# leonardsiegert/PULPo

Measured on AMD Instinct MI355X. Metric: volume-pairs/sec fwd+bwd, 160^3 fp32, higher is better.
Workload: dtype f32

## Files before the change

pulpo_amd/csrc/resample.hip:

```cpp
#include "act_io.h"

namespace {

template <int VEC, typename T = float>
__global__ __launch_bounds__(256) void avgpool2_fwd_kernel(const T* __restrict__ in, long ips, T* __restrict__ out, long ops, int B,
                                                             int D, int H, int W, int Do, int Ho, int Wo, int C) {
    const int CV = C / VEC;
    const long total = (long)B * Do * Ho * Wo * CV;
    for (long e = blockIdx.x * (long)blockDim.x + threadIdx.x; e < total; e += (long)gridDim.x * blockDim.x) {
        const int c = (int)(e % CV) * VEC;
        long p = e / CV;
        const int ox = (int)(p % Wo); p /= Wo;
        const int oy = (int)(p % Ho); p /= Ho;
        const int oz = (int)(p % Do);
        const int b = (int)(p / Do);
        const int z1 = min(2 * oz + 2, D), y1 = min(2 * oy + 2, H), x1 = min(2 * ox + 2, W);
        float acc[VEC];
#pragma unroll
        for (int k = 0; k < VEC; ++k) acc[k] = 0.f;
        for (int z = 2 * oz; z < z1; ++z)
            for (int y = 2 * oy; y < y1; ++y)
                for (int x = 2 * ox; x < x1; ++x) {
                    float t[VEC];
                    pulpo::ldv<VEC>(in + ((((long)b * D + z) * H + y) * W + x) * ips + c, t);
// ... 161 lines not shown
        const int z = (int)(p % Di);
        const long pl = p / Di;
        int zl, zh, yl, yh, xl, xh;
        gather_window(z, sd, Do, zl, zh);
        gather_window(y, sh, Ho, yl, yh);
        gather_window(x, sw, Wo, xl, xh);
        const float* g = gout + pl * (long)Do * Ho * Wo;
        float acc = 0.f;
        for (int oz = zl; oz <= zh; ++oz) {
            const float wz = gather_weight(oz, z, sd, Di);
            if (wz == 0.f) continue;
            for (int oy = yl; oy <= yh; ++oy) {
                const float wy = gather_weight(oy, y, sh, Hi);
                if (wy == 0.f) continue;
                float row = 0.f;
                for (int ox = xl; ox <= xh; ++ox) {
                    const float wx = gather_weight(ox, x, sw, Wi);
                    if (wx != 0.f) row += g[((long)oz * Ho + oy) * Wo + ox] * mult * wx;
                }
                acc += row * (wz * wy);
            }
        }
        gin[e] = acc;
    }
}

__device__ __forceinline__ float up2_weight(int o, int m, int in_size) {
    int i0, i1;
    float lam;
    src_index(o, 0.5f, in_size, i0, i1, lam);
    return (i0 == m ? 1.f - lam : 0.f) + (i1 == m ? lam : 0.f);
}

__global__ __launch_bounds__(256) void resize_up2_bwd_kernel(const float* __restrict__ gout, float* __restrict__ gin, long nplanes, int Di, int Hi,
                                                               int Wi, float mult) {
    const int Do = 2 * Di, Ho = 2 * Hi, Wo = 2 * Wi;
    const long total = nplanes * Di * Hi * Wi;
    for (long e = blockIdx.x * (long)blockDim.x + threadIdx.x; e < total; e += (long)gridDim.x * blockDim.x) {
        long p = e;
        const int x = (int)(p % Wi); p /= Wi;
        const int y = (int)(p % Hi); p /= Hi;
        const int z = (int)(p % Di);
        const long pl = p / Di;
        const float* g = gout + pl * (long)Do * Ho * Wo;
        float wz4[4], wy4[4], wx4[4];
#pragma unroll
        for (int k = 0; k < 4; ++k) {
            const int oz = 2 * z - 1 + k, oy = 2 * y - 1 + k, ox = 2 * x - 1 + k;
            wz4[k] = (oz >= 0 && oz < Do) ? up2_weight(oz, z, Di) : 0.f;
            wy4[k] = (oy >= 0 && oy < Ho) ? up2_weight(oy, y, Hi) : 0.f;
            wx4[k] = (ox >= 0 && ox < Wo) ? up2_weight(ox, x, Wi) : 0.f;
        }
        float acc = 0.f;
#pragma unroll
        for (int kz = 0; kz < 4; ++kz) {
            const int oz = 2 * z - 1 + kz;
            if (oz < 0 || oz >= Do) continue;
#pragma unroll
            for (int ky = 0; ky < 4; ++ky) {
                const int oy = 2 * y - 1 + ky;
                if (oy < 0 || oy >= Ho) continue;
                const float wzy = wz4[kz] * wy4[ky];
                const float* row = g + ((long)oz * Ho + oy) * Wo;
#pragma unroll
                for (int kx = 0; kx < 4; ++kx) {
                    const int ox = 2 * x - 1 + kx;
                    if (ox >= 0 && ox < Wo) acc += wzy * wx4[kx] * row[ox];
                }
            }
        }
        gin[e] = acc * mult;
    }
}

constexpr int kMaxSrc = 8;
struct FeedbackArgs {
    const float* src[kMaxSrc];
    float* gsrc[kMaxSrc];
    int ch[kMaxSrc];
    int nsrc, ctot;
    int B, Di, Hi, Wi;
};

template <typename T = float>
__global__ __launch_bounds__(256) void feedback_fwd_kernel(FeedbackArgs a, T* __restrict__ out, long ops) {
    const int Do = 2 * a.Di, Ho = 2 * a.Hi, Wo = 2 * a.Wi;
    const long Vi = (long)a.Di * a.Hi * a.Wi;
    const long total = (long)a.B * Do * Ho * Wo;
    for (long e = blockIdx.x * (long)blockDim.x + threadIdx.x; e < total; e += (long)gridDim.x * blockDim.x) {
        long p = e;
        const int ox = (int)(p % Wo); p /= Wo;
        const int oy = (int)(p % Ho); p /= Ho;
        const int oz = (int)(p % Do);
        const int b = (int)(p / Do);
        int z0, z1, y0, y1, x0, x1;
        float lz, ly, lx;
        src_index(oz, 0.5f, a.Di, z0, z1, lz);
        src_index(oy, 0.5f, a.Hi, y0, y1, ly);
        src_index(ox, 0.5f, a.Wi, x0, x1, lx);
        const long o00 = ((long)z0 * a.Hi + y0) * a.Wi, o01 = ((long)z0 * a.Hi + y1) * a.Wi;
        const long o10 = ((long)z1 * a.Hi + y0) * a.Wi, o11 = ((long)z1 * a.Hi + y1) * a.Wi;
        const float wz0 = 1.f - lz, wy0 = 1.f - ly, wx0 = 1.f - lx;
        T* d = out + e * ops;
        int cc = 0;
        for (int s = 0; s < a.nsrc; ++s) {
// ... 176 lines not shown
                                     int C, void* stream) {
    PULPO_REQUIRE(add != nullptr, "avgpool2_bwd_add: null pointer");
    return pulpo_avgpool2_bwd_t(gout, gops, add, aps, gin, gips, 0, B, D, H, W, C, stream);
}

PULPO_API int pulpo_resize_trilinear_scaled_fwd(const float* in, const float* add, float* out, int64_t nplanes, int Di, int Hi, int Wi, int Do, int Ho,
                                                int Wo, float scale_d, float scale_h, float scale_w, float mult, void* stream) {
    PULPO_REQUIRE(in && out && nplanes > 0 && Di > 0 && Hi > 0 && Wi > 0 && Do > 0 && Ho > 0 && Wo > 0, "resize_fwd: bad arguments");
    const float sd = scale_d > 0.f ? scale_d : (float)Di / (float)Do, sh = scale_h > 0.f ? scale_h : (float)Hi / (float)Ho,
                sw = scale_w > 0.f ? scale_w : (float)Wi / (float)Wo;
    if (Do == 2 * Di && Ho == 2 * Hi && Wo == 2 * Wi && sd == 0.5f && sh == 0.5f && sw == 0.5f && nplanes * (long)Do * Ho < (1L << 31) &&
        (((uintptr_t)out | (uintptr_t)add) & 7) == 0) {
        hipLaunchKernelGGL(resize_up2_fwd_kernel, dim3(eblocks(nplanes * Do * Ho * Wi)), dim3(256), 0, (hipStream_t)stream, in, add, out, (int)nplanes, Di, Hi,
                           Wi, mult);
        return pulpo::check_launch("resize_up2_fwd");
    }
    hipLaunchKernelGGL(resize_fwd_kernel, dim3(eblocks(nplanes * Do * Ho * Wo)), dim3(256), 0, (hipStream_t)stream, in, add, out, (long)nplanes, Di,
                       Hi, Wi, Do, Ho, Wo, sd, sh, sw, mult);
    return pulpo::check_launch("resize_fwd");
}

PULPO_API int pulpo_resize_trilinear_fwd(const float* in, const float* add, float* out, int64_t nplanes, int Di, int Hi, int Wi, int Do, int Ho, int Wo,
                                         float mult, void* stream) {
    return pulpo_resize_trilinear_scaled_fwd(in, add, out, nplanes, Di, Hi, Wi, Do, Ho, Wo, 0.f, 0.f, 0.f, mult, stream);
}

static int resize_bwd_impl(const float* gout, float* gin, int64_t nplanes, int Di, int Hi, int Wi, int Do, int Ho, int Wo,
                           float scale_d, float scale_h, float scale_w, float mult, bool det, void* stream) {
    PULPO_REQUIRE(gout && gin && nplanes > 0 && Di > 0 && Hi > 0 && Wi > 0 && Do > 0 && Ho > 0 && Wo > 0, "resize_bwd: bad arguments");
    hipStream_t st = (hipStream_t)stream;
    const float sd = scale_d > 0.f ? scale_d : (float)Di / (float)Do, sh = scale_h > 0.f ? scale_h : (float)Hi / (float)Ho,
                sw = scale_w > 0.f ? scale_w : (float)Wi / (float)Wo;
    if (Do == 2 * Di && Ho == 2 * Hi && Wo == 2 * Wi && sd == 0.5f && sh == 0.5f && sw == 0.5f) {
        hipLaunchKernelGGL(resize_up2_bwd_kernel, dim3(eblocks(nplanes * Di * Hi * Wi)), dim3(256), 0, st, gout, gin, (long)nplanes, Di, Hi, Wi, mult);
        return pulpo::check_launch("resize_up2_bwd");
    }
    if (det) {
        hipLaunchKernelGGL(resize_bwd_gather_kernel, dim3(eblocks(nplanes * Di * Hi * Wi)), dim3(256), 0, st, gout, gin, (long)nplanes, Di, Hi, Wi, Do,
                           Ho, Wo, sd, sh, sw, mult);
        return pulpo::check_launch("resize_bwd_gather");
    }
    hipError_t e = hipMemsetAsync(gin, 0, sizeof(float) * nplanes * Di * Hi * Wi, st);
    if (e != hipSuccess) return pulpo::fail((int)e, "resize_bwd memset: %s", hipGetErrorString(e));
    hipLaunchKernelGGL(resize_bwd_atomic_kernel, dim3(eblocks(nplanes * Do * Ho * Wo)), dim3(256), 0, st, gout, gin, (long)nplanes, Di, Hi, Wi, Do,
                       Ho, Wo, sd, sh, sw, mult);
    return pulpo::check_launch("resize_bwd_atomic");
}

PULPO_API int pulpo_resize_trilinear_scaled_bwd(const float* gout, float* gin, int64_t nplanes, int Di, int Hi, int Wi, int Do, int Ho, int Wo,
                                                float scale_d, float scale_h, float scale_w, float mult, void* stream) {
    return resize_bwd_impl(gout, gin, nplanes, Di, Hi, Wi, Do, Ho, Wo, scale_d, scale_h, scale_w, mult, false, stream);
}

PULPO_API int pulpo_resize_trilinear_scaled_bwd_det(const float* gout, float* gin, int64_t nplanes, int Di, int Hi, int Wi, int Do, int Ho, int Wo,
                                                    float scale_d, float scale_h, float scale_w, float mult, void* stream) {
    return resize_bwd_impl(gout, gin, nplanes, Di, Hi, Wi, Do, Ho, Wo, scale_d, scale_h, scale_w, mult, true, stream);
}

PULPO_API int pulpo_resize_trilinear_bwd(const float* gout, float* gin, int64_t nplanes, int Di, int Hi, int Wi, int Do, int Ho, int Wo, float mult,
                                         void* stream) {
    return pulpo_resize_trilinear_scaled_bwd(gout, gin, nplanes, Di, Hi, Wi, Do, Ho, Wo, 0.f, 0.f, 0.f, mult, stream);
}

PULPO_API int pulpo_feedback_up2_fwd_t(const float* const* srcs, const int* chans, int nsrc, void* out, int dt, int64_t ops, int B, int Di, int Hi,
                                       int Wi, void* stream) {
    PULPO_REQUIRE(srcs && chans && out && nsrc > 0 && nsrc <= kMaxSrc && B > 0, "feedback_up2_fwd: bad arguments");
    PULPO_REQUIRE_DT(dt, "feedback_up2_fwd");
// ... 37 lines not shown
```

pulpo_amd/csrc/warp.hip:

```cpp
#include "common.h"
#include "sampling.h"

namespace {

using pulpo::Corner;
using pulpo::sample_coord;

template <int C>
__global__ __launch_bounds__(256) void warp_fwd_kernel(const float* __restrict__ df, const float* __restrict__ img, const float* __restrict__ add,
                                                         float* __restrict__ out, int B, int Dg, int Hg, int Wg, int Di, int Hi, int Wi, int Cr) {
    const long Vg = (long)Dg * Hg * Wg, Vi = (long)Di * Hi * Wi;
    const long total = (long)B * Vg;
    const int nch = C > 0 ? C : Cr;
    for (long e = blockIdx.x * (long)blockDim.x + threadIdx.x; e < total; e += (long)gridDim.x * blockDim.x) {
        const long b = B == 1 ? 0 : e / Vg, v = e - b * Vg;
        const int vi = (int)v;
        const int x = vi % Wg, y = (vi / Wg) % Hg, z = vi / (Wg * Hg);
        const float* d = df + b * 3 * Vg + v;
        const Corner cz = sample_coord((float)z, d[0], Dg, Di);
        const Corner cy = sample_coord((float)y, d[Vg], Hg, Hi);
        const Corner cx = sample_coord((float)x, d[2 * Vg], Wg, Wi);
        const long o00 = ((long)cz.i0 * Hi + cy.i0) * Wi, o01 = ((long)cz.i0 * Hi + cy.i1) * Wi;
        const long o10 = ((long)cz.i1 * Hi + cy.i0) * Wi, o11 = ((long)cz.i1 * Hi + cy.i1) * Wi;
        const float wz0 = 1.f - cz.f, wy0 = 1.f - cy.f, wx0 = 1.f - cx.f;
// ... 197 lines not shown
                const Corner cy = sample_coord((float)y, fld[V + vox], H, H);
                const Corner cx = sample_coord((float)x, fld[2 * V + vox], W, W);
                const int o00 = (cz.i0 * H + cy.i0) * W, o01 = (cz.i0 * H + cy.i1) * W;
                const int o10 = (cz.i1 * H + cy.i0) * W, o11 = (cz.i1 * H + cy.i1) * W;
                const float wz0 = 1.f - cz.f, wy0 = 1.f - cy.f, wx0 = 1.f - cx.f;
#pragma unroll
                for (int c = 0; c < 3; ++c) {
                    const float* s = fld + c * V;
                    float val = wz0 * wy0 * wx0 * s[o00 + cx.i0] + wz0 * wy0 * cx.f * s[o00 + cx.i1] + wz0 * cy.f * wx0 * s[o01 + cx.i0] +
                                wz0 * cy.f * cx.f * s[o01 + cx.i1] + cz.f * wy0 * wx0 * s[o10 + cx.i0] + cz.f * wy0 * cx.f * s[o10 + cx.i1] +
                                cz.f * cy.f * wx0 * s[o11 + cx.i0] + cz.f * cy.f * cx.f * s[o11 + cx.i1];
                    val += s[vox];
                    nv[j][c] = val;
                }
            }
        }
        __syncthreads();
        float* out = work + (long)(k + 1) * n + b * 3 * V;
#pragma unroll
        for (int j = 0; j < 8; ++j) {
            const int vox = tid + j * VI_THREADS;
            if (vox < V) {
#pragma unroll
                for (int c = 0; c < 3; ++c) {
                    fld[c * V + vox] = nv[j][c];
                    out[c * V + vox] = nv[j][c];
                }
            }
        }
        __syncthreads();
    }
}

inline int eblocks(long items) { return (int)std::max<long>(1, std::min<long>((items + 255) / 256, 8192)); }

__device__ __forceinline__ double fx_unit(const unsigned* maxbits) {
    const float m = __uint_as_float(*maxbits);
    if (!(m > 0.f) || !(m < INFINITY)) return 1.0;
    int ex;
    frexpf(m, &ex);
    return ldexp(1.0, 46 - ex);
}
__device__ __forceinline__ void fx_add(long long* p, float v, double unit) {
    atomicAdd(reinterpret_cast<unsigned long long*>(p), (unsigned long long)__double2ll_rn((double)v * unit));
}

__device__ __forceinline__ void block_absmax_to(float m, unsigned* out) {
    __shared__ float wm[4];
#pragma unroll
    for (int o = 32; o > 0; o >>= 1) m = fmaxf(m, __shfl_xor(m, o, 64));
    if ((threadIdx.x & 63) == 0) wm[threadIdx.x >> 6] = m;
    __syncthreads();
    if (threadIdx.x == 0) {
        const float t = fmaxf(fmaxf(wm[0], wm[1]), fmaxf(wm[2], wm[3]));
        if (t > 0.f) atomicMax(out, __float_as_uint(t));
    }
}
inline int fx_blocks(long items) { return (int)std::max<long>(1, std::min<long>((items + 255) / 256, 1024)); }

__global__ __launch_bounds__(256) void absmax_kernel(const float* __restrict__ g, long n, unsigned* __restrict__ out) {
    float m = 0.f;
    for (long e = blockIdx.x * (long)blockDim.x + threadIdx.x; e < n; e += (long)gridDim.x * blockDim.x) m = fmaxf(m, fabsf(g[e]));
    block_absmax_to(m, out);
}

template <bool SELF>
// ... 98 lines not shown
    hipStream_t st = (hipStream_t)stream;
    const long n = (long)B * 3 * D * H * W, total = (long)B * D * H * W;
    constexpr long VECINT_LDS_MAXV = 2048;
    static_assert(VECINT_LDS_MAXV <= VI_MAXV, "the one-launch form holds the whole field in LDS");
    if (total / B <= VECINT_LDS_MAXV && nsteps > 0) {
        const size_t lds = sizeof(float) * 3 * (size_t)(total / B);
        static bool attr_set = false;
        if (!attr_set) {
            hipError_t e = hipFuncSetAttribute(reinterpret_cast<const void*>(&vecint_fwd_lds_kernel), hipFuncAttributeMaxDynamicSharedMemorySize,
                                               (int)(sizeof(float) * 3 * VI_MAXV));
            if (e != hipSuccess) return pulpo::fail((int)e, "hipFuncSetAttribute(vecint_fwd_lds): %s", hipGetErrorString(e));
            attr_set = true;
        }
        hipLaunchKernelGGL(vecint_fwd_lds_kernel, dim3(B), dim3(VI_THREADS), lds, st, v, work, B, D, H, W, nsteps, 1.0f / (float)(1 << nsteps));
        return pulpo::check_launch("vecint_fwd_lds");
    }
    hipLaunchKernelGGL(scale_kernel, dim3(eblocks(n)), dim3(256), 0, st, v, work, 1.0f / (float)(1 << nsteps), n);
    int rc = pulpo::check_launch("vecint scale");
    if (rc) return rc;
    for (int k = 0; k < nsteps; ++k) {
        const float* cur = work + (long)k * n;
        hipLaunchKernelGGL(warp_fwd_kernel<3>, dim3(eblocks(total)), dim3(256), 0, st, cur, cur, cur, work + (long)(k + 1) * n, B, D, H, W, D, H, W, 3);
        rc = pulpo::check_launch("vecint step");
        if (rc) return rc;
    }
    return 0;
}

static bool vecint_bwd_tiled(int D, int H, int W) {
    constexpr int TILED_MIN = 8;
    return D >= TILED_MIN && H >= TILED_MIN && W >= TILED_MIN;
}

PULPO_API size_t pulpo_vecint_bwd_tmp_floats(int B, int D, int H, int W, int nsteps) {
    if (B <= 0 || D < 1 || H < 1 || W < 1 || nsteps <= 0) return 0;
    const size_t n = (size_t)B * 3 * D * H * W;
    return vecint_bwd_tiled(D, H, W) ? (size_t)nsteps * n : 2 * n;
}

PULPO_API int pulpo_vecint_bwd(const float* work, const float* gout, float* gin, float* tmp, int B, int D, int H, int W, int nsteps, void* stream) {
    PULPO_REQUIRE(work && gout && gin && B > 0 && D >= 1 && H > 1 && W > 1 && nsteps >= 0 && (long)D * H * W < (1L << 31), "vecint_bwd: bad arguments");
    PULPO_REQUIRE(tmp || pulpo_vecint_bwd_tmp_floats(B, D, H, W, nsteps) == 0, "vecint_bwd: scratch of pulpo_vecint_bwd_tmp_floats() floats required");
    hipStream_t st = (hipStream_t)stream;
    const long n = (long)B * 3 * D * H * W, total = (long)B * D * H * W;
    const float scale = 1.0f / (float)(1 << nsteps);
    const bool tiled = vecint_bwd_tiled(D, H, W);
    if (tiled && nsteps > 0) {
        hipError_t e = hipMemsetAsync(tmp, 0, sizeof(float) * n * nsteps, st);
        if (e != hipSuccess) return pulpo::fail((int)e, "vecint_bwd fill: %s", hipGetErrorString(e));
    }
    const float* g = gout;
    for (int k = nsteps - 1; k >= 0; --k) {
        const float* cur = work + (long)k * n;
        float* gp;
        if (tiled) {
            gp = tmp + (long)k * n;
            const int ntz = pulpo::cdiv(D, 4), nty = pulpo::cdiv(H, 8), ntx = pulpo::cdiv(W, 8);
            if (k == nsteps - 1 && (long)D * H * W >= 64L * 64 * 64)
                hipLaunchKernelGGL(vecint_bwd_tile_kernel<2>, dim3((unsigned)((long)B * ntz * nty * ntx)), dim3(256), 0, st, cur, g, gp, B, D, H, W, ntz, nty, ntx);
            else
                hipLaunchKernelGGL(vecint_bwd_tile_kernel<1>, dim3((unsigned)((long)B * ntz * nty * ntx)), dim3(256), 0, st, cur, g, gp, B, D, H, W, ntz, nty, ntx);
        } else {
            gp = tmp + (long)(k & 1) * n;
            hipError_t e = hipMemcpyAsync(gp, g, sizeof(float) * n, hipMemcpyDeviceToDevice, st);
            if (e != hipSuccess) return pulpo::fail((int)e, "vecint_bwd copy: %s", hipGetErrorString(e));
            hipLaunchKernelGGL(warp_bwd_kernel<true>, dim3(eblocks(total)), dim3(256), 0, st, cur, cur, g, gp, gp, B, D, H, W, D, H, W, 3);
        }
        int rc = pulpo::check_launch("vecint_bwd step");
        if (rc) return rc;
        g = gp;
    }
    hipLaunchKernelGGL(scale_kernel, dim3(eblocks(n)), dim3(256), 0, st, g, gin, scale, n);
    return pulpo::check_launch("vecint_bwd scale");
}

PULPO_API size_t pulpo_warp3d_bwd_det_ws_bytes(int B, int C, int Di, int Hi, int Wi) {
    if (B <= 0 || C <= 0 || Di < 1 || Hi < 1 || Wi < 1) return 0;
    return 256 + sizeof(long long) * (size_t)B * C * Di * Hi * Wi;
// ... 56 lines not shown
```

pulpo_amd/csrc/conv3d_wino3.hip:

```cpp
#include "conv_shared.h"
#include "wino3_pack.h"

namespace {

using namespace pulpo_conv;
using f32x2 = __attribute__((ext_vector_type(2))) float;

constexpr int Q_CH = 8, Q_NT = 32;
constexpr int Q_PL = HY * 4;
constexpr int Q_PLROWS = 4 * Q_PL + 2;
constexpr int Q_QROWS = 6 * Q_PLROWS;
constexpr int Q_IMG = 2 * Q_QROWS * 4;
static_assert((2 * Q_PLROWS) % 16 == 4 && (Q_QROWS * 4) % 32 == 16, "bank layout");
constexpr int Q_NITEM = 6 * HY * 4 * 2;
constexpr int Q_TAB = 3 * 512;
constexpr int Q_R = 8 * 2 * 16 * 64;
constexpr int Q_RED = 8 * 2 * Q_NT;
constexpr int Q_PART = 8 * 64 * 8;
constexpr size_t Q_LDS = (size_t)(2 * Q_IMG + Q_TAB + Q_R + Q_RED + Q_PART) * sizeof(float);
static_assert(Q_LDS <= 160 * 1024, "one workgroup per CU");


template <bool BNR, int SP>
__device__ __forceinline__ void wino3_body(const ConvArgs& a) {
// ... 204 lines not shown
                    acc[s0 >> 2][s0 & 3] = __builtin_amdgcn_mfma_f32_32x32x2f32(av0[s2], wv0[s2], acc[s0 >> 2][s0 & 3], 0, 0, 0);
                    acc[s1 >> 2][s1 & 3] = __builtin_amdgcn_mfma_f32_32x32x2f32(av1[s2], wv1[s2], acc[s1 >> 2][s1 & 3], 0, 0, 0);
                    if (s2 == 0) {
                        __builtin_amdgcn_sched_barrier(0);
                        if (pp == SP) {
                            store_item(img_w);
                            if (chunk + 2 == nchunk) halo_offsets(has_next ? nxt : cur);
                        }
                        if (pp == SP + 1) { load_raw(st_rs, st_c0, 0); load_raw(st_rs, st_c0, 1); load_raw(st_rs, st_c0, 2); load_raw(st_rs, st_c0, 3); }
                        __builtin_amdgcn_sched_barrier(0);
                    }
                    if (s2 == 1 && pp + 1 < 4) {
                        __builtin_amdgcn_sched_barrier(0);
                        combine(avn0, avn1);
                        __builtin_amdgcn_sched_barrier(0);
                        if (pp + 2 < 4) fetch_a(pp + 2);
                        __builtin_amdgcn_sched_barrier(0);
                    }
                }
                wr[pp & 1][0] = pp < 2 ? load_w(wcur, s0 + 2) : load_w(wnext, s0 - 2);
                wr[pp & 1][1] = pp < 2 ? load_w(wcur, s1 + 2) : load_w(wnext, s1 - 2);
                __builtin_amdgcn_sched_barrier(0);
            }
            wcur += w_chunk_stride;
            __syncthreads();
            cb ^= 1;
            if (chunk == 0) flush_stats();
        }

        float* out_b = a.out + (long)cur.b * a.out_bs;
        const int z0 = cur.z0, y0 = cur.y0, x0 = cur.x0, co0 = cur.co0;
        int elane = lane;
        asm volatile("" : "+v"(elane));
        const int q = elane & 7, kh = (elane >> 3) & 1, g = elane >> 4;
        const float4 zero4 = make_float4(0.f, 0.f, 0.f, 0.f);
        float4 s4 = zero4, q4 = zero4;
        const bool fuse = !BNR && a.coef != nullptr;
        const float4 b4 = BNR ? zero4 : *reinterpret_cast<const float4*>(tab + co0 + 4 * q);
        const float4 bm4 = *reinterpret_cast<const float4*>(tab + co0 + 4 * q);
        const float4 sc4 = *reinterpret_cast<const float4*>(tab + ctab + co0 + 4 * q);
        const float4 sh4 = *reinterpret_cast<const float4*>(tab + 2 * ctab + co0 + 4 * q);
        const float* bn_b = BNR ? a.bn_y + (long)cur.b * a.bn_y_bs + co0 + 4 * q : nullptr;
        const int combo = wave * 4 + g;
        const int ox = combo >> 4, rr = combo & 15;
        const int row = (rr & 3) + 8 * (rr >> 2) + 4 * kh;
        const int vzb = row >> 4, vyb = (row >> 2) & 3, vxb = row & 3;
        float4 yv0 = zero4, yv1 = zero4;
        const bool qok = co0 + 4 * q < a.Cout;
        auto load_y = [&](int oz_) {
            if (BNR && qok) {
                const long vox_ = (long)((z0 + 2 * vzb + oz_) * a.H + y0 + 2 * vyb) * a.W + x0 + 2 * vxb + ox;
                yv0 = *reinterpret_cast<const float4*>(bn_b + vox_ * a.bn_y_ps);
                yv1 = *reinterpret_cast<const float4*>(bn_b + (vox_ + a.W) * a.bn_y_ps);
            }
        };
        load_y(0);
        __builtin_amdgcn_sched_barrier(0);
        f32x2 m1 = {-1.f, -1.f};
        asm volatile("" : "+s"(m1));
#pragma unroll
        for (int p = 0; p < 2; ++p)
#pragma unroll
            for (int r = 0; r < 16; r += 2) {
                const f32x2 a0 = {acc[p][0][r], acc[p][0][r + 1]}, a1 = {acc[p][1][r], acc[p][1][r + 1]};
                const f32x2 a2 = {acc[p][2][r], acc[p][2][r + 1]}, a3 = {acc[p][3][r], acc[p][3][r + 1]};
                const f32x2 o0 = (a0 + a1) + a2, o1 = __builtin_elementwise_fma(m1, a3, __builtin_elementwise_fma(m1, a2, a1));
                acc[p][0][r] = o0.x; acc[p][0][r + 1] = o0.y;
                acc[p][1][r] = o1.x; acc[p][1][r + 1] = o1.y;
            }
#pragma unroll
        for (int oz = 0; oz < 2; ++oz) {
            if (oz > 0) __syncthreads();
            float* const r0 = R + ((wave * 2 + 0) * 16) * 64 + elane;
            float* const r1 = R + ((wave * 2 + 1) * 16) * 64 + elane;
            if (pzh == 0) {
#pragma unroll
                for (int r = 0; r < 16; r += 2) {
                    const f32x2 u0 = f32x2{acc[0][0][r], acc[0][0][r + 1]} + f32x2{acc[1][0][r], acc[1][0][r + 1]};
                    const f32x2 u1 = f32x2{acc[0][1][r], acc[0][1][r + 1]} + f32x2{acc[1][1][r], acc[1][1][r + 1]};
                    r0[r * 64] = oz == 0 ? u0.x : acc[1][0][r]; r0[(r + 1) * 64] = oz == 0 ? u0.y : acc[1][0][r + 1];
                    r1[r * 64] = oz == 0 ? u1.x : acc[1][1][r]; r1[(r + 1) * 64] = oz == 0 ? u1.y : acc[1][1][r + 1];
                }
            } else {
#pragma unroll
                for (int r = 0; r < 16; r += 2) {
                    const f32x2 u0 = __builtin_elementwise_fma(m1, f32x2{acc[0][0][r], acc[0][0][r + 1]}, f32x2{acc[1][0][r], acc[1][0][r + 1]});
                    const f32x2 u1 = __builtin_elementwise_fma(m1, f32x2{acc[0][1][r], acc[0][1][r + 1]}, f32x2{acc[1][1][r], acc[1][1][r + 1]});
                    r0[r * 64] = oz == 0 ? acc[0][0][r] : u0.x; r0[(r + 1) * 64] = oz == 0 ? acc[0][0][r + 1] : u0.y;
                    r1[r * 64] = oz == 0 ? acc[0][1][r] : u1.x; r1[(r + 1) * 64] = oz == 0 ? acc[0][1][r + 1] : u1.y;
                }
            }
            const int gz = z0 + 2 * vzb + oz, gy = y0 + 2 * vyb, gx = x0 + 2 * vxb + ox;
            const long vox = (long)(gz * a.H + gy) * a.W + gx;
            __syncthreads();
            float4 t[4];
#pragma unroll
            for (int p = 0; p < 4; ++p) {
                const float4 u0 = *reinterpret_cast<const float4*>(R + (((0 * 4 + p) * 2 + ox) * 16 + rr) * 64 + kh * 32 + 4 * q);
                const float4 u1 = *reinterpret_cast<const float4*>(R + (((1 * 4 + p) * 2 + ox) * 16 + rr) * 64 + kh * 32 + 4 * q);
                t[p] = make_float4(u0.x + u1.x, u0.y + u1.y, u0.z + u1.z, u0.w + u1.w);
            }
            float4 v0 = make_float4(t[0].x + t[1].x + t[2].x + b4.x, t[0].y + t[1].y + t[2].y + b4.y, t[0].z + t[1].z + t[2].z + b4.z, t[0].w + t[1].w + t[2].w + b4.w);
            float4 v1 = make_float4(t[1].x - t[2].x - t[3].x + b4.x, t[1].y - t[2].y - t[3].y + b4.y, t[1].z - t[2].z - t[3].z + b4.z, t[1].w - t[2].w - t[3].w + b4.w);
            if (BNR) {
                auto red1 = [&](float dzv, float yy, float sc, float sh, float m32, float& s_, float& q_) {
                    const float bn = yy * sc + sh;
                    const float d = bn > 0.f ? dzv : dzv * a.slope;
                    s_ += d;
                    q_ = fmaf(d, yy - m32, q_);
                };
                red1(v0.x, yv0.x, sc4.x, sh4.x, bm4.x, s4.x, q4.x); red1(v0.y, yv0.y, sc4.y, sh4.y, bm4.y, s4.y, q4.y);
                red1(v0.z, yv0.z, sc4.z, sh4.z, bm4.z, s4.z, q4.z); red1(v0.w, yv0.w, sc4.w, sh4.w, bm4.w, s4.w, q4.w);
                red1(v1.x, yv1.x, sc4.x, sh4.x, bm4.x, s4.x, q4.x); red1(v1.y, yv1.y, sc4.y, sh4.y, bm4.y, s4.y, q4.y);
                red1(v1.z, yv1.z, sc4.z, sh4.z, bm4.z, s4.z, q4.z); red1(v1.w, yv1.w, sc4.w, sh4.w, bm4.w, s4.w, q4.w);
                if (oz == 0) { __builtin_amdgcn_sched_barrier(0); load_y(1); __builtin_amdgcn_sched_barrier(0); }
            } else {
                s4.x += v0.x + v1.x; s4.y += v0.y + v1.y; s4.z += v0.z + v1.z; s4.w += v0.w + v1.w;
                q4.x += v0.x * v0.x + v1.x * v1.x; q4.y += v0.y * v0.y + v1.y * v1.y; q4.z += v0.z * v0.z + v1.z * v1.z; q4.w += v0.w * v0.w + v1.w * v1.w;
            }
            if (fuse) {
                auto act = [&](float v, float sc, float sh) { const float tt = v * sc + sh; return tt > 0.f ? tt : tt * a.slope; };
                v0 = make_float4(act(v0.x, sc4.x, sh4.x), act(v0.y, sc4.y, sh4.y), act(v0.z, sc4.z, sh4.z), act(v0.w, sc4.w, sh4.w));
                v1 = make_float4(act(v1.x, sc4.x, sh4.x), act(v1.y, sc4.y, sh4.y), act(v1.z, sc4.z, sh4.z), act(v1.w, sc4.w, sh4.w));
            }
            float* obase = out_b + (long)((co0 + 4 * q) >> 3) * a.out_kb + ((4 * q) & 7);
            if (qok) {
                *reinterpret_cast<float4*>(obase + vox * a.out_ps) = v0;
                *reinterpret_cast<float4*>(obase + (vox + a.W) * a.out_ps) = v1;
            }
        }
        if (a.stats != nullptr) {
            float* pw_ = part + (wave * 64 + elane) * 8;
            *reinterpret_cast<float4*>(pw_) = s4;
            *reinterpret_cast<float4*>(pw_ + 4) = q4;
            const int c_ = elane & 31, wh_ = elane >> 5;
            const float* pr_ = part + (wave * 64 + (c_ >> 2)) * 8 + wh_ * 4 + (c_ & 3);
            float t_ = 0.f;
#pragma unroll
            for (int j = 0; j < 8; ++j) t_ += pr_[j * 64];
            red[(wave * 2 + wh_) * NT + c_] = t_;
        }
        pend_tile = cur.tile_lin; pend_co0 = co0;
        if (!has_next) break;
        cur = nxt;
        work = next_work;
    }
    __syncthreads();
    flush_stats();
}

template <bool BNR>
__global__ __launch_bounds__(512, 1) void conv3d_k3_wino3_mfma(ConvArgs a) {
    if (__builtin_amdgcn_readfirstlane(threadIdx.x >> 8) != 0) wino3_body<BNR, 2>(a);
    else wino3_body<BNR, 0>(a);
}

__global__ void pack_weight_wino3_kernel(const float* __restrict__ w, float* __restrict__ wp, int Cin, int Cout, int NPad, int dgrad, long total) {
    for (long e = blockIdx.x * (long)blockDim.x + threadIdx.x; e < total; e += (long)gridDim.x * blockDim.x)
        pulpo_conv::pack_wino3_one(w, wp, Cin, Cout, NPad, dgrad, e);
}

constexpr int WINO3_MIN_K = 16;

// ... 103 lines not shown
```

Baseline: 38.02.

## Tile up2 resize backward through LDS and fuse small-volume vecint backward

The 2x-upsample trilinear backward now runs one block per 4x8x8 coarse tile. Each block stages its fine-gradient halo in shared memory and gathers from there, instead of every thread issuing 64 global loads. Separately, for tiny volumes (at most 1024 voxels), the whole scaling-and-squaring backward runs in one block-per-batch kernel that keeps the field and gradients in LDS across all steps. This removes the per-step launches, the memset and the scratch buffer. The fused path only triggers for small volumes, and the tiled resize adds a barrier and halo-redundant loads.

Result: no change. 38.19, median of 6 (+0.5%).

```diff
diff --git a/pulpo_amd/csrc/resample.hip b/pulpo_amd/csrc/resample.hip
--- a/pulpo_amd/csrc/resample.hip
+++ b/pulpo_amd/csrc/resample.hip
@@ -217,45 +217,53 @@
     return (i0 == m ? 1.f - lam : 0.f) + (i1 == m ? lam : 0.f);
 }
 
-__global__ __launch_bounds__(256) void resize_up2_bwd_kernel(const float* __restrict__ gout, float* __restrict__ gin, long nplanes, int Di, int Hi,
-                                                               int Wi, float mult) {
+template <int TZ_, int TY_, int TX_>
+__global__ __launch_bounds__(TZ_* TY_* TX_) void resize_up2_bwd_kernel(const float* __restrict__ gout, float* __restrict__ gin, int Di, int Hi, int Wi,
+                                                                       int ntz, int nty, int ntx, float mult) {
+    constexpr int NT = TZ_ * TY_ * TX_, FY = 2 * TY_ + 2, FX = 2 * TX_ + 2, FV = (2 * TZ_ + 2) * FY * FX;
+    __shared__ float fine[FV];
     const int Do = 2 * Di, Ho = 2 * Hi, Wo = 2 * Wi;
-    const long total = nplanes * Di * Hi * Wi;
-    for (long e = blockIdx.x * (long)blockDim.x + threadIdx.x; e < total; e += (long)gridDim.x * blockDim.x) {
-        long p = e;
-        const int x = (int)(p % Wi); p /= Wi;
-        const int y = (int)(p % Hi); p /= Hi;
-        const int z = (int)(p % Di);
-        const long pl = p / Di;
-        const float* g = gout + pl * (long)Do * Ho * Wo;
-        float wz4[4], wy4[4], wx4[4];
-#pragma unroll
-        for (int k = 0; k < 4; ++k) {
-            const int oz = 2 * z - 1 + k, oy = 2 * y - 1 + k, ox = 2 * x - 1 + k;
-            wz4[k] = (oz >= 0 && oz < Do) ? up2_weight(oz, z, Di) : 0.f;
-            wy4[k] = (oy >= 0 && oy < Ho) ? up2_weight(oy, y, Hi) : 0.f;
-            wx4[k] = (ox >= 0 && ox < Wo) ? up2_weight(ox, x, Wi) : 0.f;
-        }
-        float acc = 0.f;
-#pragma unroll
-        for (int kz = 0; kz < 4; ++kz) {
-            const int oz = 2 * z - 1 + kz;
-            if (oz < 0 || oz >= Do) continue;
-#pragma unroll
-            for (int ky = 0; ky < 4; ++ky) {
-                const int oy = 2 * y - 1 + ky;
-                if (oy < 0 || oy >= Ho) continue;
-                const float wzy = wz4[kz] * wy4[ky];
-                const float* row = g + ((long)oz * Ho + oy) * Wo;
-#pragma unroll
-                for (int kx = 0; kx < 4; ++kx) {
-                    const int ox = 2 * x - 1 + kx;
-                    if (ox >= 0 && ox < Wo) acc += wzy * wx4[kx] * row[ox];
-                }
+    int t = blockIdx.x;
+    const int tx_ = t % ntx; t /= ntx;
+    const int ty_ = t % nty; t /= nty;
+    const int tz_ = t % ntz;
+    const long pl = t / ntz;
+    const int z0 = tz_ * TZ_, y0 = ty_ * TY_, x0 = tx_ * TX_;
+    const float* g = gout + pl * (long)Do * Ho * Wo;
+    for (int j = threadIdx.x; j < FV; j += NT) {
+        const int oz = 2 * z0 - 1 + j / (FY * FX), oy = 2 * y0 - 1 + (j / FX) % FY, ox = 2 * x0 - 1 + j % FX;
+        fine[j] = (oz >= 0 && oz < Do && oy >= 0 && oy < Ho && ox >= 0 && ox < Wo) ? g[((long)oz * Ho + oy) * Wo + ox] : 0.f;
+    }
+    __syncthreads();
+    const int z = z0 + threadIdx.x / (TY_ * TX_), y = y0 + (threadIdx.x / TX_) % TY_, x = x0 + threadIdx.x % TX_;
+    if (z >= Di || y >= Hi || x >= Wi) return;
+    float wz4[4], wy4[4], wx4[4];
+#pragma unroll
+    for (int k = 0; k < 4; ++k) {
+        const int oz = 2 * z - 1 + k, oy = 2 * y - 1 + k, ox = 2 * x - 1 + k;
+        wz4[k] = (oz >= 0 && oz < Do) ? up2_weight(oz, z, Di) : 0.f;
+        wy4[k] = (oy >= 0 && oy < Ho) ? up2_weight(oy, y, Hi) : 0.f;
+        wx4[k] = (ox >= 0 && ox < Wo) ? up2_weight(ox, x, Wi) : 0.f;
+    }
+    float acc = 0.f;
+#pragma unroll
+    for (int kz = 0; kz < 4; ++kz) {
+        const int oz = 2 * z - 1 + kz;
+        if (oz < 0 || oz >= Do) continue;
+#pragma unroll
+        for (int ky = 0; ky < 4; ++ky) {
+            const int oy = 2 * y - 1 + ky;
+            if (oy < 0 || oy >= Ho) continue;
+            const float wzy = wz4[kz] * wy4[ky];
+            const float* row = fine + ((2 * (z - z0) + kz) * FY + 2 * (y - y0) + ky) * FX + 2 * (x - x0);
+#pragma unroll
+            for (int kx = 0; kx < 4; ++kx) {
+                const int ox = 2 * x - 1 + kx;
+                if (ox >= 0 && ox < Wo) acc += wzy * wx4[kx] * row[kx];
             }
         }
-        gin[e] = acc * mult;
-    }
+    }
+    gin[((pl * Di + z) * Hi + y) * (long)Wi + x] = acc * mult;
 }
 
 constexpr int kMaxSrc = 8;
@@ -498,7 +506,11 @@
     const float sd = scale_d > 0.f ? scale_d : (float)Di / (float)Do, sh = scale_h > 0.f ? scale_h : (float)Hi / (float)Ho,
                 sw = scale_w > 0.f ? scale_w : (float)Wi / (float)Wo;
     if (Do == 2 * Di && Ho == 2 * Hi && Wo == 2 * Wi && sd == 0.5f && sh == 0.5f && sw == 0.5f) {
-        hipLaunchKernelGGL(resize_up2_bwd_kernel, dim3(eblocks(nplanes * Di * Hi * Wi)), dim3(256), 0, st, gout, gin, (long)nplanes, Di, Hi, Wi, mult);
+        constexpr int TZ = 4, TY = 8, TX = 8;
+        const int ntz = pulpo::cdiv(Di, TZ), nty = pulpo::cdiv(Hi, TY), ntx = pulpo::cdiv(Wi, TX);
+        PULPO_REQUIRE(nplanes * ntz * nty * ntx < (1L << 31), "resize_bwd: too many tiles");
+        hipLaunchKernelGGL((resize_up2_bwd_kernel<TZ, TY, TX>), dim3((unsigned)(nplanes * ntz * nty * ntx)), dim3(TZ * TY * TX), 0, st, gout, gin, Di, Hi, Wi,
+                           ntz, nty, ntx, mult);
         return pulpo::check_launch("resize_up2_bwd");
     }
     if (det) {
diff --git a/pulpo_amd/csrc/warp.hip b/pulpo_amd/csrc/warp.hip
--- a/pulpo_amd/csrc/warp.hip
+++ b/pulpo_amd/csrc/warp.hip
@@ -253,6 +253,126 @@
     }
 }
 
+constexpr int VB_THREADS = 1024;
+__global__ __launch_bounds__(VB_THREADS) void vecint_bwd_lds_kernel(const float* __restrict__ work, const float* __restrict__ gout, float* __restrict__ gin,
+                                                                      int B, int D, int H, int W, int nsteps, float scale) {
+    __shared__ float fld[3 * VB_THREADS];
+    __shared__ float gs[3 * VB_THREADS];
+    __shared__ float wt[9 * VB_THREADS];
+    const int V = D * H * W, tid = threadIdx.x;
+    const long b = blockIdx.x, n = (long)B * 3 * V;
+    const bool valid = tid < V;
+    const int x = tid % W, y = (tid / W) % H, z = tid / (W * H);
+    float d0 = 0.f, d1 = 0.f, d2 = 0.f;
+    if (valid) {
+#pragma unroll
+        for (int c = 0; c < 3; ++c) gs[c * V + tid] = gout[b * 3 * V + c * V + tid];
+        const float* cur = work + (long)(nsteps - 1) * n + b * 3 * V;
+        d0 = cur[tid];
+        d1 = cur[V + tid];
+        d2 = cur[2 * V + tid];
+    }
+    for (int k = nsteps - 1; k >= 0; --k) {
+        Corner cz = {0, 0, 0.f, 0.f}, cy = cz, cx = cz;
+        bool far = false;
+        if (valid) {
+            fld[tid] = d0;
+            fld[V + tid] = d1;
+            fld[2 * V + tid] = d2;
+            cz = sample_coord((float)z, d0, D, D);
+            cy = sample_coord((float)y, d1, H, H);
+            cx = sample_coord((float)x, d2, W, W);
+            const int ez = cz.i0 - z, ey = cy.i0 - y, ex = cx.i0 - x;
+            far = !(ez >= -1 && ez <= 0 && ey >= -1 && ey <= 0 && ex >= -1 && ex <= 0);
+            float w[9];
+#pragma unroll
+            for (int i = 0; i < 9; ++i) w[i] = 0.f;
+            if (!far) {
+                w[1 - ez] = 1.f - cz.f;
+                w[-ez] = cz.f;
+                w[4 - ey] = 1.f - cy.f;
+                w[3 - ey] = cy.f;
+                w[7 - ex] = 1.f - cx.f;
+                w[6 - ex] = cx.f;
+            }
+#pragma unroll
+            for (int i = 0; i < 9; ++i) wt[i * V + tid] = w[i];
+        }
+        __syncthreads();
+        if (valid && k > 0) {
+            const float* nxt = work + (long)(k - 1) * n + b * 3 * V;
+            d0 = nxt[tid];
+            d1 = nxt[V + tid];
+            d2 = nxt[2 * V + tid];
+        }
+        const float wz0 = 1.f - cz.f, wy0 = 1.f - cy.f, wx0 = 1.f - cx.f;
+        const int o00 = (cz.i0 * H + cy.i0) * W, o01 = (cz.i0 * H + cy.i1) * W;
+        const int o10 = (cz.i1 * H + cy.i0) * W, o11 = (cz.i1 * H + cy.i1) * W;
+        float acc[3] = {0.f, 0.f, 0.f}, gown[3] = {0.f, 0.f, 0.f};
+        if (valid) {
+            float gz = 0.f, gy = 0.f, gx = 0.f;
+#pragma unroll
+            for (int c = 0; c < 3; ++c) {
+                const float g = gs[c * V + tid];
+                gown[c] = g;
+                const float* s = fld + c * V;
+                const float s000 = s[o00 + cx.i0], s001 = s[o00 + cx.i1], s010 = s[o01 + cx.i0], s011 = s[o01 + cx.i1];
+                const float s100 = s[o10 + cx.i0], s101 = s[o10 + cx.i1], s110 = s[o11 + cx.i0], s111 = s[o11 + cx.i1];
+                gz += g * (wy0 * wx0 * (s100 - s000) + wy0 * cx.f * (s101 - s001) + cy.f * wx0 * (s110 - s010) + cy.f * cx.f * (s111 - s011));
+                gy += g * (wz0 * wx0 * (s010 - s000) + wz0 * cx.f * (s011 - s001) + cz.f * wx0 * (s110 - s100) + cz.f * cx.f * (s111 - s101));
+                gx += g * (wz0 * wy0 * (s001 - s000) + wz0 * cy.f * (s011 - s010) + cz.f * wy0 * (s101 - s100) + cz.f * cy.f * (s111 - s110));
+            }
+            acc[0] = gown[0] + gz * cz.dscale;
+            acc[1] = gown[1] + gy * cy.dscale;
+            acc[2] = gown[2] + gx * cx.dscale;
+#pragma unroll 1
+            for (int oz = -1; oz <= 1; ++oz) {
+                if (z + oz < 0 || z + oz >= D) continue;
+#pragma unroll
+                for (int oy = -1; oy <= 1; ++oy) {
+                    if (y + oy < 0 || y + oy >= H) continue;
+#pragma unroll
+                    for (int ox = -1; ox <= 1; ++ox) {
+                        if (x + ox < 0 || x + ox >= W) continue;
+                        const int j = tid + (oz * H + oy) * W + ox;
+                        const float w = wt[(1 + oz) * V + j] * wt[(4 + oy) * V + j] * wt[(7 + ox) * V + j];
+                        acc[0] += gs[j] * w;
+                        acc[1] += gs[V + j] * w;
+                        acc[2] += gs[2 * V + j] * w;
+                    }
+                }
+            }
+        }
+        __syncthreads();
+        if (valid) {
+#pragma unroll
+            for (int c = 0; c < 3; ++c) gs[c * V + tid] = acc[c];
+        }
+        if (__syncthreads_or(far)) {
+            if (far) {
+#pragma unroll
+                for (int c = 0; c < 3; ++c) {
+                    const float g = gown[c];
+                    float* q = gs + c * V;
+                    atomicAdd(q + o00 + cx.i0, g * wz0 * wy0 * wx0);
+                    atomicAdd(q + o00 + cx.i1, g * wz0 * wy0 * cx.f);
+                    atomicAdd(q + o01 + cx.i0, g * wz0 * cy.f * wx0);
+                    atomicAdd(q + o01 + cx.i1, g * wz0 * cy.f * cx.f);
+                    atomicAdd(q + o10 + cx.i0, g * cz.f * wy0 * wx0);
+                    atomicAdd(q + o10 + cx.i1, g * cz.f * wy0 * cx.f);
+                    atomicAdd(q + o11 + cx.i0, g * cz.f * cy.f * wx0);
+                    atomicAdd(q + o11 + cx.i1, g * cz.f * cy.f * cx.f);
+                }
+            }
+            __syncthreads();
+        }
+    }
+    if (valid) {
+#pragma unroll
+        for (int c = 0; c < 3; ++c) gin[b * 3 * V + c * V + tid] = gs[c * V + tid] * scale;
+    }
+}
+
 inline int eblocks(long items) { return (int)std::max<long>(1, std::min<long>((items + 255) / 256, 8192)); }
 
 __device__ __forceinline__ double fx_unit(const unsigned* maxbits) {
@@ -417,8 +537,10 @@
     return D >= TILED_MIN && H >= TILED_MIN && W >= TILED_MIN;
 }
 
+static bool vecint_bwd_one_launch(int D, int H, int W) { return vecint_bwd_tiled(D, H, W) && (long)D * H * W <= VB_THREADS; }
+
 PULPO_API size_t pulpo_vecint_bwd_tmp_floats(int B, int D, int H, int W, int nsteps) {
-    if (B <= 0 || D < 1 || H < 1 || W < 1 || nsteps <= 0) return 0;
+    if (B <= 0 || D < 1 || H < 1 || W < 1 || nsteps <= 0 || vecint_bwd_one_launch(D, H, W)) return 0;
     const size_t n = (size_t)B * 3 * D * H * W;
     return vecint_bwd_tiled(D, H, W) ? (size_t)nsteps * n : 2 * n;
 }
@@ -429,6 +551,10 @@
     hipStream_t st = (hipStream_t)stream;
     const long n = (long)B * 3 * D * H * W, total = (long)B * D * H * W;
     const float scale = 1.0f / (float)(1 << nsteps);
+    if (vecint_bwd_one_launch(D, H, W) && nsteps > 0) {
+        hipLaunchKernelGGL(vecint_bwd_lds_kernel, dim3(B), dim3(VB_THREADS), 0, st, work, gout, gin, B, D, H, W, nsteps, scale);
+        return pulpo::check_launch("vecint_bwd_lds");
+    }
     const bool tiled = vecint_bwd_tiled(D, H, W);
     if (tiled && nsteps > 0) {
         hipError_t e = hipMemsetAsync(tmp, 0, sizeof(float) * n * nsteps, st);
```

## Restructure Winograd epilogue: interleave inverse transform with LDS stores, packed f32x2 math

Applied to the files above, without the earlier changes.

Rewrites the Winograd output epilogue so the x-inverse transform is interleaved with the LDS staging writes. The second z-plane is staged right after the first plane's reads instead of in a separate loop iteration. The bias, BN-backward reduction, activation and stats math are converted to packed f32x2 operations. Addresses are precomputed once per tile, and the oz offset is handled with a plane stride. The aim is to cut VALU instruction count and overlap LDS traffic with arithmetic, at the cost of more live registers and tighter scheduling constraints.

Result: no change. 38.13 before, 38.08 after (-0.1%).

```diff
diff --git a/pulpo_amd/csrc/conv3d_wino3.hip b/pulpo_amd/csrc/conv3d_wino3.hip
--- a/pulpo_amd/csrc/conv3d_wino3.hip
+++ b/pulpo_amd/csrc/conv3d_wino3.hip
@@ -260,103 +260,148 @@
         const int z0 = cur.z0, y0 = cur.y0, x0 = cur.x0, co0 = cur.co0;
         int elane = lane;
         asm volatile("" : "+v"(elane));
+        const float4 zero4 = make_float4(0.f, 0.f, 0.f, 0.f);
+        const bool fuse = !BNR && a.coef != nullptr;
+        int eW = a.W, eH = a.H;
+        if (BNR) asm volatile("" : "+s"(eW), "+s"(eH));
+        const long vrow = eW, vpl = (long)eH * eW;
+        auto lane_vox0 = [&](int el) {
+            const int combo = wave * 4 + (el >> 4);
+            const int ox = combo >> 4, rr = combo & 15;
+            const int row = (rr & 3) + 8 * (rr >> 2) + 4 * ((el >> 3) & 1);
+            const int vzb = row >> 4, vyb = (row >> 2) & 3, vxb = row & 3;
+            return (long)((z0 + 2 * vzb) * eH + y0 + 2 * vyb) * eW + x0 + 2 * vxb + ox;
+        };
+        float4 yv0 = zero4, yv1 = zero4;
+        auto load_y = [&](int el, int oz_) {
+            if (BNR && co0 + 4 * (el & 7) < a.Cout) {
+                const float* yb = a.bn_y + (long)cur.b * a.bn_y_bs + co0 + 4 * (el & 7) + lane_vox0(el) * a.bn_y_ps;
+                yv0 = *reinterpret_cast<const float4*>(yb + oz_ * vpl * a.bn_y_ps);
+                yv1 = *reinterpret_cast<const float4*>(yb + (oz_ * vpl + vrow) * a.bn_y_ps);
+            }
+        };
+        load_y(elane, 0);
+        __builtin_amdgcn_sched_barrier(0);
+        f32x2 m1 = {-1.f, -1.f};
+        asm volatile("" : "+s"(m1));
+        auto xinv = [&](int p, int r) {
+            const f32x2 a0 = {acc[p][0][r], acc[p][0][r + 1]}, a1 = {acc[p][1][r], acc[p][1][r + 1]};
+            const f32x2 a2 = {acc[p][2][r], acc[p][2][r + 1]}, a3 = {acc[p][3][r], acc[p][3][r + 1]};
+            const f32x2 o0 = (a0 + a1) + a2, o1 = __builtin_elementwise_fma(m1, a3, __builtin_elementwise_fma(m1, a2, a1));
+            acc[p][0][r] = o0.x; acc[p][0][r + 1] = o0.y;
+            acc[p][1][r] = o1.x; acc[p][1][r + 1] = o1.y;
+        };
+        float* const r0 = R + ((wave * 2 + 0) * 16) * 64 + elane;
+        float* const r1 = R + ((wave * 2 + 1) * 16) * 64 + elane;
+        auto put = [&](int r, const f32x2 u0, const f32x2 u1) {
+            r0[r * 64] = u0.x; r0[(r + 1) * 64] = u0.y;
+            r1[r * 64] = u1.x; r1[(r + 1) * 64] = u1.y;
+        };
+        if (pzh == 0) {
+#pragma unroll
+            for (int r = 0; r < 16; r += 2) {
+                xinv(0, r); xinv(1, r);
+                put(r, f32x2{acc[0][0][r], acc[0][0][r + 1]} + f32x2{acc[1][0][r], acc[1][0][r + 1]},
+                    f32x2{acc[0][1][r], acc[0][1][r + 1]} + f32x2{acc[1][1][r], acc[1][1][r + 1]});
+                __builtin_amdgcn_sched_barrier(0);
+            }
+        } else {
+#pragma unroll
+            for (int r = 0; r < 16; r += 2) {
+                xinv(0, r);
+                put(r, f32x2{acc[0][0][r], acc[0][0][r + 1]}, f32x2{acc[0][1][r], acc[0][1][r + 1]});
+                __builtin_amdgcn_sched_barrier(0);
+            }
+#pragma unroll
+            for (int r = 0; r < 16; r += 2) xinv(1, r);
+        }
+        auto put1 = [&]() {
+            if (pzh == 0) {
+#pragma unroll
+                for (int r = 0; r < 16; r += 2) put(r, f32x2{acc[1][0][r], acc[1][0][r + 1]}, f32x2{acc[1][1][r], acc[1][1][r + 1]});
+            } else {
+#pragma unroll
+                for (int r = 0; r < 16; r += 2)
+                    put(r, __builtin_elementwise_fma(m1, f32x2{acc[0][0][r], acc[0][0][r + 1]}, f32x2{acc[1][0][r], acc[1][0][r + 1]}),
+                        __builtin_elementwise_fma(m1, f32x2{acc[0][1][r], acc[0][1][r + 1]}, f32x2{acc[1][1][r], acc[1][1][r + 1]}));
+            }
+        };
+        __builtin_amdgcn_sched_barrier(0);
+        asm volatile("" : "+v"(elane));
         const int q = elane & 7, kh = (elane >> 3) & 1, g = elane >> 4;
-        const float4 zero4 = make_float4(0.f, 0.f, 0.f, 0.f);
-        float4 s4 = zero4, q4 = zero4;
-        const bool fuse = !BNR && a.coef != nullptr;
+        const int combo = wave * 4 + g;
+        const int ox = combo >> 4, rr = combo & 15;
+        const bool qok = co0 + 4 * q < a.Cout;
+        const long vox0 = lane_vox0(elane);
+        const float* const rd = R + (ox * 16 + rr) * 64 + kh * 32 + 4 * q;
+        f32x2 tl[4], th[4];
+        auto read_t = [&]() {
+            float4 u[2][4];
+#pragma unroll
+            for (int p = 0; p < 4; ++p) {
+                u[0][p] = *reinterpret_cast<const float4*>(rd + ((0 * 4 + p) * 2 * 16) * 64);
+                u[1][p] = *reinterpret_cast<const float4*>(rd + ((1 * 4 + p) * 2 * 16) * 64);
+            }
+            __builtin_amdgcn_sched_barrier(0);
+#pragma unroll
+            for (int p = 0; p < 4; ++p) {
+                tl[p] = f32x2{u[0][p].x, u[0][p].y} + f32x2{u[1][p].x, u[1][p].y};
+                th[p] = f32x2{u[0][p].z, u[0][p].w} + f32x2{u[1][p].z, u[1][p].w};
+            }
+        };
         const float4 b4 = BNR ? zero4 : *reinterpret_cast<const float4*>(tab + co0 + 4 * q);
         const float4 bm4 = *reinterpret_cast<const float4*>(tab + co0 + 4 * q);
         const float4 sc4 = *reinterpret_cast<const float4*>(tab + ctab + co0 + 4 * q);
         const float4 sh4 = *reinterpret_cast<const float4*>(tab + 2 * ctab + co0 + 4 * q);
-        const float* bn_b = BNR ? a.bn_y + (long)cur.b * a.bn_y_bs + co0 + 4 * q : nullptr;
-        const int combo = wave * 4 + g;
-        const int ox = combo >> 4, rr = combo & 15;
-        const int row = (rr & 3) + 8 * (rr >> 2) + 4 * kh;
-        const int vzb = row >> 4, vyb = (row >> 2) & 3, vxb = row & 3;
-        float4 yv0 = zero4, yv1 = zero4;
-        const bool qok = co0 + 4 * q < a.Cout;
-        auto load_y = [&](int oz_) {
-            if (BNR && qok) {
-                const long vox_ = (long)((z0 + 2 * vzb + oz_) * a.H + y0 + 2 * vyb) * a.W + x0 + 2 * vxb + ox;
-                yv0 = *reinterpret_cast<const float4*>(bn_b + vox_ * a.bn_y_ps);
-                yv1 = *reinterpret_cast<const float4*>(bn_b + (vox_ + a.W) * a.bn_y_ps);
-            }
-        };
-        load_y(0);
+        long o00_ = (long)((co0 + 4 * q) >> 3) * a.out_kb + ((4 * q) & 7) + vox0 * a.out_ps;
+        const f32x2 bl = {b4.x, b4.y}, bh = {b4.z, b4.w}, bml = {bm4.x, bm4.y}, bmh = {bm4.z, bm4.w};
+        const f32x2 scl = {sc4.x, sc4.y}, sch = {sc4.z, sc4.w}, shl = {sh4.x, sh4.y}, shh = {sh4.z, sh4.w};
+        const f32x2 slope2 = {a.slope, a.slope};
+        f32x2 sl = {0.f, 0.f}, sh_ = {0.f, 0.f}, ql = {0.f, 0.f}, qh = {0.f, 0.f};
+        asm volatile("" : "+v"(o00_));
+        float* const o00 = out_b + o00_;
+        __syncthreads();
         __builtin_amdgcn_sched_barrier(0);
-        f32x2 m1 = {-1.f, -1.f};
-        asm volatile("" : "+s"(m1));
-#pragma unroll
-        for (int p = 0; p < 2; ++p)
-#pragma unroll
-            for (int r = 0; r < 16; r += 2) {
-                const f32x2 a0 = {acc[p][0][r], acc[p][0][r + 1]}, a1 = {acc[p][1][r], acc[p][1][r + 1]};
-                const f32x2 a2 = {acc[p][2][r], acc[p][2][r + 1]}, a3 = {acc[p][3][r], acc[p][3][r + 1]};
-                const f32x2 o0 = (a0 + a1) + a2, o1 = __builtin_elementwise_fma(m1, a3, __builtin_elementwise_fma(m1, a2, a1));
-                acc[p][0][r] = o0.x; acc[p][0][r + 1] = o0.y;
-                acc[p][1][r] = o1.x; acc[p][1][r + 1] = o1.y;
-            }
-#pragma unroll
-        for (int oz = 0; oz < 2; ++oz) {
-            if (oz > 0) __syncthreads();
-            float* const r0 = R + ((wave * 2 + 0) * 16) * 64 + elane;
-            float* const r1 = R + ((wave * 2 + 1) * 16) * 64 + elane;
-            if (pzh == 0) {
-#pragma unroll
-                for (int r = 0; r < 16; r += 2) {
-                    const f32x2 u0 = f32x2{acc[0][0][r], acc[0][0][r + 1]} + f32x2{acc[1][0][r], acc[1][0][r + 1]};
-                    const f32x2 u1 = f32x2{acc[0][1][r], acc[0][1][r + 1]} + f32x2{acc[1][1][r], acc[1][1][r + 1]};
-                    r0[r * 64] = oz == 0 ? u0.x : acc[1][0][r]; r0[(r + 1) * 64] = oz == 0 ? u0.y : acc[1][0][r + 1];
-                    r1[r * 64] = oz == 0 ? u1.x : acc[1][1][r]; r1[(r + 1) * 64] = oz == 0 ? u1.y : acc[1][1][r + 1];
-                }
+        read_t();
+        auto lrelu = [&](const f32x2 c, const f32x2 pos, const f32x2 neg) { return f32x2{c.x > 0.f ? pos.x : neg.x, c.y > 0.f ? pos.y : neg.y}; };
+        auto finish = [&](int oz_) {
+            f32x2 v0l = ((tl[0] + tl[1]) + tl[2]) + bl, v0h = ((th[0] + th[1]) + th[2]) + bh;
+            f32x2 v1l = __builtin_elementwise_fma(m1, tl[3], __builtin_elementwise_fma(m1, tl[2], tl[1])) + bl;
+            f32x2 v1h = __builtin_elementwise_fma(m1, th[3], __builtin_elementwise_fma(m1, th[2], th[1])) + bh;
+            if (BNR) {
+                auto red2 = [&](const f32x2 dzv, const f32x2 yy, const f32x2 sc, const f32x2 sh, const f32x2 m32, f32x2& s_, f32x2& q_) {
+                    const f32x2 bn = __builtin_elementwise_fma(yy, sc, sh);
+                    const f32x2 d = lrelu(bn, dzv, dzv * slope2);
+                    s_ = s_ + d;
+                    q_ = __builtin_elementwise_fma(d, __builtin_elementwise_fma(m1, m32, yy), q_);
+                };
+                red2(v0l, f32x2{yv0.x, yv0.y}, scl, shl, bml, sl, ql); red2(v0h, f32x2{yv0.z, yv0.w}, sch, shh, bmh, sh_, qh);
+                red2(v1l, f32x2{yv1.x, yv1.y}, scl, shl, bml, sl, ql); red2(v1h, f32x2{yv1.z, yv1.w}, sch, shh, bmh, sh_, qh);
+                if (oz_ == 0) { __builtin_amdgcn_sched_barrier(0); load_y(elane, 1); __builtin_amdgcn_sched_barrier(0); }
             } else {
-#pragma unroll
-                for (int r = 0; r < 16; r += 2) {
-                    const f32x2 u0 = __builtin_elementwise_fma(m1, f32x2{acc[0][0][r], acc[0][0][r + 1]}, f32x2{acc[1][0][r], acc[1][0][r + 1]});
-                    const f32x2 u1 = __builtin_elementwise_fma(m1, f32x2{acc[0][1][r], acc[0][1][r + 1]}, f32x2{acc[1][1][r], acc[1][1][r + 1]});
-                    r0[r * 64] = oz == 0 ? acc[0][0][r] : u0.x; r0[(r + 1) * 64] = oz == 0 ? acc[0][0][r + 1] : u0.y;
-                    r1[r * 64] = oz == 0 ? acc[0][1][r] : u1.x; r1[(r + 1) * 64] = oz == 0 ? acc[0][1][r + 1] : u1.y;
-                }
-            }
-            const int gz = z0 + 2 * vzb + oz, gy = y0 + 2 * vyb, gx = x0 + 2 * vxb + ox;
-            const long vox = (long)(gz * a.H + gy) * a.W + gx;
-            __syncthreads();
-            float4 t[4];
-#pragma unroll
-            for (int p = 0; p < 4; ++p) {
-                const float4 u0 = *reinterpret_cast<const float4*>(R + (((0 * 4 + p) * 2 + ox) * 16 + rr) * 64 + kh * 32 + 4 * q);
-                const float4 u1 = *reinterpret_cast<const float4*>(R + (((1 * 4 + p) * 2 + ox) * 16 + rr) * 64 + kh * 32 + 4 * q);
-                t[p] = make_float4(u0.x + u1.x, u0.y + u1.y, u0.z + u1.z, u0.w + u1.w);
-            }
-            float4 v0 = make_float4(t[0].x + t[1].x + t[2].x + b4.x, t[0].y + t[1].y + t[2].y + b4.y, t[0].z + t[1].z + t[2].z + b4.z, t[0].w + t[1].w + t[2].w + b4.w);
-            float4 v1 = make_float4(t[1].x - t[2].x - t[3].x + b4.x, t[1].y - t[2].y - t[3].y + b4.y, t[1].z - t[2].z - t[3].z + b4.z, t[1].w - t[2].w - t[3].w + b4.w);
-            if (BNR) {
-                auto red1 = [&](float dzv, float yy, float sc, float sh, float m32, float& s_, float& q_) {
-                    const float bn = yy * sc + sh;
-                    const float d = bn > 0.f ? dzv : dzv * a.slope;
-                    s_ += d;
-                    q_ = fmaf(d, yy - m32, q_);
-                };
-                red1(v0.x, yv0.x, sc4.x, sh4.x, bm4.x, s4.x, q4.x); red1(v0.y, yv0.y, sc4.y, sh4.y, bm4.y, s4.y, q4.y);
-                red1(v0.z, yv0.z, sc4.z, sh4.z, bm4.z, s4.z, q4.z); red1(v0.w, yv0.w, sc4.w, sh4.w, bm4.w, s4.w, q4.w);
-                red1(v1.x, yv1.x, sc4.x, sh4.x, bm4.x, s4.x, q4.x); red1(v1.y, yv1.y, sc4.y, sh4.y, bm4.y, s4.y, q4.y);
-                red1(v1.z, yv1.z, sc4.z, sh4.z, bm4.z, s4.z, q4.z); red1(v1.w, yv1.w, sc4.w, sh4.w, bm4.w, s4.w, q4.w);
-                if (oz == 0) { __builtin_amdgcn_sched_barrier(0); load_y(1); __builtin_amdgcn_sched_barrier(0); }
-            } else {
-                s4.x += v0.x + v1.x; s4.y += v0.y + v1.y; s4.z += v0.z + v1.z; s4.w += v0.w + v1.w;
-                q4.x += v0.x * v0.x + v1.x * v1.x; q4.y += v0.y * v0.y + v1.y * v1.y; q4.z += v0.z * v0.z + v1.z * v1.z; q4.w += v0.w * v0.w + v1.w * v1.w;
+                sl = sl + (v0l + v1l); sh_ = sh_ + (v0h + v1h);
+                ql = ql + __builtin_elementwise_fma(v0l, v0l, v1l * v1l); qh = qh + __builtin_elementwise_fma(v0h, v0h, v1h * v1h);
             }
             if (fuse) {
-                auto act = [&](float v, float sc, float sh) { const float tt = v * sc + sh; return tt > 0.f ? tt : tt * a.slope; };
-                v0 = make_float4(act(v0.x, sc4.x, sh4.x), act(v0.y, sc4.y, sh4.y), act(v0.z, sc4.z, sh4.z), act(v0.w, sc4.w, sh4.w));
-                v1 = make_float4(act(v1.x, sc4.x, sh4.x), act(v1.y, sc4.y, sh4.y), act(v1.z, sc4.z, sh4.z), act(v1.w, sc4.w, sh4.w));
-            }
-            float* obase = out_b + (long)((co0 + 4 * q) >> 3) * a.out_kb + ((4 * q) & 7);
+                auto act = [&](const f32x2 v, const f32x2 sc, const f32x2 sh) { const f32x2 tt = __builtin_elementwise_fma(v, sc, sh); return lrelu(tt, tt, tt * slope2); };
+                v0l = act(v0l, scl, shl); v0h = act(v0h, sch, shh);
+                v1l = act(v1l, scl, shl); v1h = act(v1h, sch, shh);
+            }
             if (qok) {
-                *reinterpret_cast<float4*>(obase + vox * a.out_ps) = v0;
-                *reinterpret_cast<float4*>(obase + (vox + a.W) * a.out_ps) = v1;
-            }
-        }
+                *reinterpret_cast<float4*>(o00 + oz_ * vpl * a.out_ps) = make_float4(v0l.x, v0l.y, v0h.x, v0h.y);
+                *reinterpret_cast<float4*>(o00 + (oz_ * vpl + vrow) * a.out_ps) = make_float4(v1l.x, v1l.y, v1h.x, v1h.y);
+            }
+        };
+        __builtin_amdgcn_sched_barrier(0);
+        __syncthreads();
+        put1();
+        __builtin_amdgcn_sched_barrier(0);
+        finish(0);
+        __builtin_amdgcn_sched_barrier(0);
+        __syncthreads();
+        read_t();
+        finish(1);
+        const float4 s4 = make_float4(sl.x, sl.y, sh_.x, sh_.y), q4 = make_float4(ql.x, ql.y, qh.x, qh.y);
         if (a.stats != nullptr) {
             float* pw_ = part + (wave * 64 + elane) * 8;
             *reinterpret_cast<float4*>(pw_) = s4;
```
